# JzHuai0108/sim3opt

Hardware: AMD Instinct MI355X
Metric: LM iterations/s (higher is better)
Workload: dtype f64

## Files before the change

sim3opt_amd/csrc/amg_kernels.hpp:

```cpp
#pragma once

__global__ __launch_bounds__(WG) void k_amg_adjoint(int nb, const int32_t* __restrict__ row2v,
                                                    const Sim3* __restrict__ states,
                                                    double* __restrict__ P) {
  for (int i = blockIdx.x * WG + threadIdx.x; i < nb; i += gridDim.x * WG) {
  const Sim3 S = load_sim3(states + row2v[i]);
  double R[9];
  sim3::R_from_quat(S.q, R);
  double A[49];
#pragma unroll
  for (int k = 0; k < 49; ++k) A[k] = 0.0;
  const double t0 = S.t[0], t1 = S.t[1], t2 = S.t[2];
#pragma unroll
  for (int c = 0; c < 3; ++c) {
    const double v0 = R[c], v1 = R[3 + c], v2 = R[6 + c];
    A[0 + 7 * c] = v0;
    A[1 + 7 * c] = v1;
    A[2 + 7 * c] = v2;
    A[3 + 7 * c] = t1 * v2 - t2 * v1;
    A[4 + 7 * c] = t2 * v0 - t0 * v2;
    A[5 + 7 * c] = t0 * v1 - t1 * v0;
    A[3 + 7 * (3 + c)] = S.s * v0;
    A[4 + 7 * (3 + c)] = S.s * v1;
    A[5 + 7 * (3 + c)] = S.s * v2;
  }
  A[3 + 42] = -t0;
  A[4 + 42] = -t1;
  A[5 + 42] = -t2;
  A[6 + 42] = 1.0;
  double* dst = P + (size_t)49 * i;
#pragma unroll
  for (int k = 0; k < 49; ++k) dst[k] = A[k];
  }
}

template <bool HASP>
__global__ __launch_bounds__(WG) void k_amg_galerkin(int cb0, int cb1, const int32_t* __restrict__ gptr,
                                                     const int32_t* __restrict__ gblk,
                                                     const int32_t* __restrict__ grow,
                                                     const int32_t* __restrict__ colidx_f,
                                                     const double* __restrict__ vals_f,
                                                     const double* __restrict__ P,
                                                     double* __restrict__ vals_c,
                                                     float* __restrict__ vals32_f) {
  const int lane = threadIdx.x & 63;
  const int cb = cb0 + __builtin_amdgcn_readfirstlane((int)(blockIdx.x * 4 + (threadIdx.x >> 6)));
  if (cb >= cb1) return;
  const int l49 = lane < 49 ? lane : lane - 49;
  const int r = l49 % 7, c = l49 / 7;
  double acc = 0.0;
  const int e0 = gptr[cb], e1 = gptr[cb + 1];
  for (int eb = e0; eb < e1; eb += 64) {
    const int n = e1 - eb < 64 ? e1 - eb : 64;
    const int le = lane < n ? lane : n - 1;
    const int kkv = gblk[eb + le];
    if (HASP) {
      const int giv = grow[eb + le];
      const int cjv = colidx_f[kkv];
      double av[2], pj[2][7], pi[2][7];
      int kk[2];
      auto load = [&](int u, int b) {
        kk[b] = __builtin_amdgcn_readlane(kkv, u);
        av[b] = vals_f[(size_t)49 * kk[b] + l49];
        const double* pjp = P + (size_t)49 * __builtin_amdgcn_readlane(cjv, u) + 7 * c;
        const double* pip = P + (size_t)49 * __builtin_amdgcn_readlane(giv, u) + 7 * r;
#pragma unroll
        for (int q = 0; q < 7; ++q) {
          pj[b][q] = pjp[q];
          pi[b][q] = pip[q];
        }
      };
      auto consume = [&](int b) {
        if (vals32_f && lane < 49) vals32_f[f32_pair_index(kk[b], lane)] = (float)av[b];
        double t = 0.0;
#pragma unroll
        for (int q = 0; q < 7; ++q) t += __shfl(av[b], r + 7 * q) * pj[b][q];
        double o = 0.0;
#pragma unroll
        for (int q = 0; q < 7; ++q) o += pi[b][q] * __shfl(t, q + 7 * c);
        acc += o;
      };
      for (int u = 0; u < n; ++u) {
        load(u, 0);
        consume(0);
      }
    } else {
      for (int u0 = 0; u0 < n; u0 += 4) {
        const int m = n - u0 < 4 ? n - u0 : 4;
        int kk[4];
        double av[4];
#pragma unroll
        for (int u = 0; u < 4; ++u)
          if (u < m) {
            kk[u] = __builtin_amdgcn_readlane(kkv, u0 + u);
            av[u] = vals_f[(size_t)49 * kk[u] + l49];
          }
#pragma unroll
        for (int u = 0; u < 4; ++u)
          if (u < m) {
            if (vals32_f && lane < 49) vals32_f[f32_pair_index(kk[u], lane)] = (float)av[u];
            acc += av[u];
          }
      }
    }
  }
  if (lane < 49) vals_c[(size_t)49 * cb + lane] = acc;
}

__global__ __launch_bounds__(WG) void k_amg_copydiag(int lo, int hi, const int32_t* __restrict__ rowptr,
                                                     const double* __restrict__ vals,
                                                     double* __restrict__ diagH) {
  for (int idx = 49 * lo + blockIdx.x * WG + threadIdx.x; idx < 49 * hi; idx += gridDim.x * WG)
    diagH[idx] = vals[(size_t)49 * rowptr[idx / 49] + idx % 49];
}

// ... 19 lines not shown
      acc += v;
    }
  }
  if (lane < 49) Wc[(size_t)49 * a + lane] = acc;
}


template <int K>
__global__ __launch_bounds__(WG) void k_amg_restrict(int a_lo, int nc, const int32_t* __restrict__ mptr,
                                                     const int32_t* __restrict__ mem,
                                                     const double* __restrict__ t_f,
                                                     double* __restrict__ r_c,
                                                     const double* __restrict__ Minv_c,
                                                     double* __restrict__ x_c, int64_t vs_f, int64_t vs_c,
                                                     int64_t ms_c) {
  const int lane = threadIdx.x & 63;
  const int wave = threadIdx.x >> 6;
  const int sub = lane / 7, rr = lane % 7, base = lane - rr;
  if (gridDim.y > 1) {
    const size_t s0 = (size_t)blockIdx.y * K;
    t_f += s0 * vs_f;
    r_c += s0 * vs_c;
    x_c += s0 * vs_c;
    if (Minv_c) Minv_c += s0 * ms_c;
  }
  for (int a0 = a_lo + (blockIdx.x * 4 + wave) * 9; a0 < nc; a0 += gridDim.x * 36) {
    const int a = a0 + sub;
    const bool act = lane < 63 && a < nc;
    const int e0 = act ? mptr[a] : 0, e1 = act ? mptr[a + 1] : 0;
#pragma unroll
    for (int s = 0; s < K; ++s) {
      const double* tf = t_f + (size_t)s * vs_f;
      double acc = 0.0;
      int e = e0;
      for (; e + 3 < e1; e += 4) {
        const int i0 = mem[e], i1 = mem[e + 1], i2 = mem[e + 2], i3 = mem[e + 3];
        const double v0 = tf[(size_t)7 * i0 + rr], v1 = tf[(size_t)7 * i1 + rr];
        const double v2 = tf[(size_t)7 * i2 + rr], v3 = tf[(size_t)7 * i3 + rr];
        acc += (v0 + v1) + (v2 + v3);
      }
      for (; e < e1; ++e) acc += tf[(size_t)7 * mem[e] + rr];
      if (act) r_c[(size_t)s * vs_c + (size_t)7 * a + rr] = acc;
      if (Minv_c) {
        double xv = 0.0;
#pragma unroll
        for (int cc = 0; cc < 7; ++cc) {
          const double rc = __shfl(acc, base + cc);
          if (act) xv += Minv_c[(size_t)s * ms_c + (size_t)49 * a + 7 * rr + cc] * rc;
        }
        if (act) x_c[(size_t)s * vs_c + (size_t)7 * a + rr] = xv;
      }
    }
  }
}

template <int K>
__device__ inline bool all_done(const DevScalars* __restrict__ sc) {
  bool done = sc != nullptr;
#pragma unroll
  for (int s = 0; s < K; ++s) done = done && sc[s].done;
  return done;
}

template <int K>
__global__ __launch_bounds__(WG) void k_amg_restrict0(int a_lo, int nc, const int32_t* __restrict__ mptr,
                                                      const int32_t* __restrict__ mem,
                                                      const double* __restrict__ P,
                                                      const double* __restrict__ t_f,
                                                      double* __restrict__ r_c,
                                                      const double* __restrict__ Minv_c,
                                                      double* __restrict__ x_c,
                                                      const DevScalars* __restrict__ sc, int64_t vs_f, int64_t vs_c,
                                                      int64_t ms_c) {
  if (all_done<K>(sc)) return;
  const int lane = threadIdx.x & 63;
  const int a = a_lo + __builtin_amdgcn_readfirstlane((int)(blockIdx.x * 4 + (threadIdx.x >> 6)));
  if (a >= nc) return;
  const int l49 = lane < 49 ? lane : lane - 49;
  const int m = l49 % 7, c = l49 / 7;
  double acc[K];
#pragma unroll
  for (int s = 0; s < K; ++s) acc[s] = 0.0;
  const int e0 = mptr[a], e1 = mptr[a + 1];
  for (int e = e0; e < e1; ++e) {
    const int i = mem[e];
    const double pv = P[(size_t)49 * i + l49];
#pragma unroll
    for (int s = 0; s < K; ++s) acc[s] += pv * t_f[(size_t)s * vs_f + (size_t)7 * i + m];
  }
#pragma unroll
  for (int s = 0; s < K; ++s) {
    double rc = 0.0;
#pragma unroll
    for (int q = 0; q < 7; ++q) rc += __shfl(acc[s], 7 * c + q);
    if (lane < 49 && m == 0) r_c[(size_t)s * vs_c + (size_t)7 * a + c] = rc;
    if (Minv_c) {
      const double pr = Minv_c[(size_t)s * ms_c + (size_t)49 * a + l49] * rc;
      double xv = pr;
#pragma unroll
      for (int q = 1; q < 7; ++q) xv += __shfl(pr, m + 7 * ((c + q) % 7));
      if (lane < 7) x_c[(size_t)s * vs_c + (size_t)7 * a + lane] = xv;
    }
  }
}

__global__ __launch_bounds__(WG) void k_amg_bjapply(int nb, const double* __restrict__ Minv,
                                                    const double* __restrict__ r,
                                                    double* __restrict__ x) {
  const int lane = threadIdx.x & 63;
  const int wave = threadIdx.x >> 6;
  const int sub = lane / 7, rr = lane % 7, base = lane - rr;
  for (int row0 = (blockIdx.x * 4 + wave) * 9; row0 < nb; row0 += gridDim.x * 36) {
    const int row = row0 + sub;
    const bool act = lane < 63 && row < nb;
    const double rv = act ? r[(size_t)7 * row + rr] : 0.0;
    double xv = 0.0;
#pragma unroll
    for (int cc = 0; cc < 7; ++cc) {
      const double rc = __shfl(rv, base + cc);
      if (act) xv += Minv[(size_t)49 * row + 7 * rr + cc] * rc;
    }
    if (act) x[(size_t)7 * row + rr] = xv;
  }
}

template <bool HASP, int K>
__global__ __launch_bounds__(WG) void k_amg_prolong(int row_lo, int row_hi, const int32_t* __restrict__ list,
                                                    const int32_t* __restrict__ agg,
                                                    const double* __restrict__ P,
                                                    const double* __restrict__ x_c,
                                                    const double* x_in, double* x_out,
                                                    const DevScalars* __restrict__ sc, double scale, int64_t vs_f,
                                                    int64_t vs_c) {
  if (all_done<K>(sc)) return;
  const int lane = threadIdx.x & 63;
  const int wave = threadIdx.x >> 6;
  const int sub = lane / 7, rr = lane % 7, base = lane - rr;
  for (int row0 = row_lo + (blockIdx.x * 4 + wave) * 9; row0 < row_hi; row0 += gridDim.x * 36) {
    const bool act = lane < 63 && row0 + sub < row_hi;
    const int row = act ? (list ? list[row0 + sub] : row0 + sub) : 0;
    const int ag = act ? agg[row] : 0;
    constexpr bool HOIST = HASP && K > 1;
    double pm[HOIST ? 7 : 1];
    if constexpr (HOIST) {
#pragma unroll
      for (int m = 0; m < 7; ++m) pm[m] = act ? P[(size_t)49 * row + rr + 7 * m] : 0.0;
    }
#pragma unroll
    for (int s = 0; s < K; ++s) {
      const double xc = act ? x_c[(size_t)s * vs_c + (size_t)7 * ag + rr] : 0.0;
      double add = xc;
      if constexpr (HASP) {
        add = 0.0;
#pragma unroll
        for (int m = 0; m < 7; ++m) {
          const double xm = __shfl(xc, base + m);
          if constexpr (HOIST) {
            if (act) add += pm[m] * xm;
          } else {
            if (act) add += P[(size_t)49 * row + rr + 7 * m] * xm;
          }
        }
      }
      const size_t j = (size_t)s * vs_f + (size_t)7 * row + rr;
      if (act) x_out[j] = x_in[j] + scale * add;
    }
  }
}

constexpr int AMG_DENSE_MAX_N = 7 * AMG_MAX_COARSEST;
__global__ __launch_bounds__(WG) void k_amg_dense_fill(int nb, const int32_t* __restrict__ rowptr,
                                                       const int32_t* __restrict__ colidx,
                                                       const double* __restrict__ vals,
                                                       double* __restrict__ A,
                                                       const double* __restrict__ diag64 = nullptr) {
  const int n = 7 * nb;
  const int nnz = 49 * rowptr[nb];
  for (int t = blockIdx.x * WG + threadIdx.x; t < nnz; t += gridDim.x * WG) {
    const int k = t / 49, e = t % 49;
    int lo = 0, hi = nb;
    while (hi - lo > 1) {
      const int mid = (lo + hi) >> 1;
      if (rowptr[mid] <= k) lo = mid; else hi = mid;
    }
    const double v = diag64 && k == rowptr[lo] ? diag64[(size_t)49 * lo + e] : vals[(size_t)49 * k + e];
    A[(size_t)(7 * lo + e % 7) * n + 7 * colidx[k] + e / 7] = v;
  }
}


template <int NP>
__device__ inline bool gj_invert_rows(double (&prow)[NP], int lane) {
  bool spd = true;
#pragma unroll
  for (int k = 0; k < NP; ++k) {
    double pk[NP];
#pragma unroll
    for (int c = 0; c < NP; ++c) pk[c] = __shfl(prow[c], k);
    if (!(pk[k] > 0.0)) spd = false;
    const double d = 1.0 / pk[k];
    const double f = prow[k];
#pragma unroll
    for (int j = 0; j < NP; ++j) {
      const double rk = pk[j] * d;
      if (lane == k) prow[j] = j == k ? d : rk;
      else prow[j] = j == k ? -f * d : prow[j] - f * rk;
    }
  }
  return spd;
}

template <int NP>
__device__ inline bool gj_invert_halfrows(double (&prow)[NP / 2], int lane) {
  constexpr int H = NP / 2;
  const int r = lane & 31, h = lane >> 5;
  bool spd = true;
#pragma unroll
  for (int k = 0; k < NP; ++k) {
    const int hk = k / H, kk = k % H;
    double pk[H];
#pragma unroll
    for (int c = 0; c < H; ++c) pk[c] = __shfl(prow[c], k + 32 * h);
    const double pkk = __shfl(prow[kk], k + 32 * hk);
    if (!(pkk > 0.0)) spd = false;
    const double d = 1.0 / pkk;
    const double f = __shfl(prow[kk], r + 32 * hk);
#pragma unroll
    for (int j = 0; j < H; ++j) {
      const double rk = pk[j] * d;
      const bool pivcol = j == kk && h == hk;
      if (r == k) prow[j] = pivcol ? d : rk;
      else prow[j] = pivcol ? -f * d : prow[j] - f * rk;
    }
  }
  return spd;
}

template <int NP>
__device__ inline void gj_invert_block(const double* src, int ld, double* __restrict__ Pout, int lane,
                                       DevScalars* sc) {
  bool spd;
  if constexpr (NP % 2 == 0) {
    constexpr int H = NP / 2;
    double prow[H];
// ... 166 lines not shown
```

sim3opt_amd/csrc/engine_amg.hip:

```cpp
#include "engine_impl.hpp"

#include <cassert>

namespace sim3opt {

#include "spmv_kernel.hpp"
#include "amg_kernels.hpp"

int Engine::amg_init(const Structure& s, bool automatic, std::string& err) {
  (void)err;
  amg_omega = std::max(0.1, std::min(0.95, opt.amg_omega));
  amg_additive = opt.amg_additive != 0;
  {
    const bool partitioned = part_world() >= 2;
    int last = 0;
    for (int l = 1; l <= AMG_MAX_LEVELS; ++l) {
      const int o = l <= 4 ? opt.amg_cycle[l - 1] : 0;
      if (o >= 1 && o <= 3) last = o;
      amg_visits[l] = last > 0 ? last : (partitioned ? (l <= 1 ? 1 : 2) : (l <= 1 ? 2 : 3));
    }
    amg_visits[0] = 1;
  }
  amg_fp32 = opt.amg_fp32 != 0;
  adaptive_prec = opt.adaptive_prec != 0 && automatic;
  amg_pivot = opt.amg_pivot >= 28 ? 28 : 14;
  for (int l = 0; l <= AMG_MAX_LEVELS; ++l)
    amg_over_l[l] = std::max(0.5, std::min(3.0, l == 0 ? opt.amg_over[0] : opt.amg_over[1]));
  std::string why;
  AmgBuildOptions bo;
  bo.max_coarsest = opt.amg_coarsest;
  for (int k = 0; k < 3; ++k) bo.passes[k] = opt.amg_passes[k];
  std::vector<int32_t> vbegin;
  bo.world = part_world();
  bo.shard_rows = std::max(1, opt.amg_shard_rows);
  if (comm.world > 1) {
    bo.row_begin = row_begin.data();
  } else if (bo.world > 1) {
    vbegin.resize(bo.world + 1);
    partition_rows_equal(nb, bo.world, vbegin.data());
    bo.row_begin = vbegin.data();
  }
  if (!build_amg_hierarchy(nb, s.rowptr.data(), s.colidx.data(), amg_host, why, bo)) {
    if (opt.verbose) std::fprintf(stderr, "sim3opt: no multigrid hierarchy (%s)\n", why.c_str());
    amg_host.clear();
    return SIM3OPT_OK;
  }
  if (automatic && (double)amg_host[1].nnzb > 0.3 * (double)amg_host[0].nnzb) {
    if (opt.verbose)
      std::fprintf(stderr, "sim3opt: the graph coarsens like an expander (level-1 blocks %.2f of level 0): block-Jacobi\n",
                   (double)amg_host[1].nnzb / (double)amg_host[0].nnzb);
    amg_host.clear();
    return SIM3OPT_OK;
  }
  use_amg = true;
  return SIM3OPT_OK;
}

int Engine::amg_bind(const Structure& s, std::string& err) {
  std::vector<AmgLevelHost>& H = amg_host;
  const int nl = (int)H.size();
  amg.assign(nl, AmgLevel());
  int rc = SIM3OPT_OK;
#define AMGCHK(call) do { rc = (call); if (rc) return rc; } while (0)
  AmgLevel& L0 = amg[0];
  L0.nb = nb; L0.nnzb = nnzb;
  L0.rowptr = d_rowptr; L0.colidx = d_colidx; L0.wrow = d_wrow; L0.span_grid = span_grid;
  L0.vals = d_vals; L0.Minv = d_Minv; L0.r = d_r; L0.x = d_z;
  int64_t padded = 0;
  (void)allgather_equal_plan(offs.data(), comm.world, nullptr, &padded);
  HIPCHK(mem.alloc(d_az, std::max<size_t>((size_t)n, (size_t)padded), nullptr));
  HIPCHK(mem.alloc(d_P, (size_t)49 * nb, nullptr));
  HIPCHK(upload(d_row2v, s.row2vertex));
  L0.t = d_az;
  L0.lo = r0; L0.hi = r1;
  const int64_t shard_rows = std::max(1, opt.amg_shard_rows);
  rep_level = 1;
  while (rep_level < nl - 1 && H[rep_level].nb > shard_rows && !H[rep_level].row_begin.empty() &&
         H[rep_level].respects_owner)
    ++rep_level;
  if (comm.active()) {
    parts.resize(rep_level);
    n_sharded = rep_level;
  }
  for (int l = 0; l < nl; ++l) {
    AmgLevel& L = amg[l];
    const AmgLevelHost& h = H[l];
    if (l > 0) {
      L.nb = h.nb; L.nnzb = h.nnzb;
      L.lo = 0; L.hi = L.nb;
      HIPCHK(upload(L.rowptr, h.rowptr));
      HIPCHK(upload(L.colidx, h.colidx));
      if (sharded(l)) {
        AMGCHK(level_part_init(l, L.nb, h.rowptr.data(), h.colidx.data(), h.row_begin, err));
        L.lo = parts[l].lo; L.hi = parts[l].hi;
      }
      const int nloc = L.hi - L.lo;
      L.span_grid = std::max(1, (nloc + 3) / 4);
      std::vector<int32_t> wrow(L.span_grid * 4 + 1);
      partition_rows(nloc, h.rowptr.data() + L.lo, L.span_grid * 4, wrow.data());
      for (int32_t& w : wrow) w += L.lo;
      HIPCHK(upload(L.wrow, wrow));
      AMGCHK(alloc_ranged(L.vals, 49 * (int64_t)h.rowptr[L.lo], 49 * (int64_t)h.rowptr[L.hi], 49 * (int64_t)L.nnzb, err));
      HIPCHK(mem.alloc(L.diagH, (size_t)49 * L.nb, nullptr));
      HIPCHK(mem.alloc(L.W, (size_t)49 * L.nb, nullptr));
      HIPCHK(mem.alloc(L.Minv, (size_t)49 * L.nb, nullptr));
      HIPCHK(mem.alloc(L.r, (size_t)7 * L.nb, nullptr));
      HIPCHK(mem.alloc(L.x, (size_t)7 * L.nb, nullptr));
      HIPCHK(mem.alloc(L.t, (size_t)7 * L.nb, nullptr));
    }
    if (amg_fp32) {
      const int64_t b0 = l == 0 ? s.rowptr[L.lo] : h.rowptr[L.lo], b1 = l == 0 ? s.rowptr[L.hi] : h.rowptr[L.hi];
      const int64_t n32 = 98 * ((std::max<int64_t>(L.nnzb, 1) + 1) / 2);
      AMGCHK(alloc_ranged(L.vals32, 98 * (b0 / 2), 98 * ((b1 + 1) / 2), n32, err));
    }
    if (l + 1 < nl) {
      HIPCHK(upload(L.agg, h.agg));
      HIPCHK(upload(L.mptr, h.mptr));
      HIPCHK(upload(L.mem, h.mem));
      HIPCHK(upload(L.gptr, h.gptr));
      HIPCHK(upload(L.gblk, h.gblk));
      HIPCHK(upload(L.grow, h.grow));
    }
  }
  const size_t nc = (size_t)7 * amg[nl - 1].nb;
  HIPCHK(mem.alloc(d_Ainv, nc * nc, nullptr));
  HIPCHK(mem.alloc(d_Ainv2, nc * nc, nullptr));
  HIPCHK(mem.alloc(d_piv, 2 * 28 * 28, nullptr));
#undef AMGCHK
  lvl_offs.assign(nl, std::vector<int64_t>());
  lvl_blk_offs.assign(nl, std::vector<int64_t>());
  for (int l = 1; l < nl; ++l) {
    amg[l].own_lo = 0; amg[l].own_hi = amg[l].nb;
    if (sharded(l - 1)) {
      const std::vector<int32_t> rb = H[l].row_begin.empty() ? std::vector<int32_t>{0, H[l].nb} : H[l].row_begin;
      amg[l].own_lo = rb[comm.rank];
      amg[l].own_hi = rb[comm.rank + 1];
      lvl_offs[l].resize(comm.world + 1);
      lvl_blk_offs[l].resize(comm.world + 1);
      for (int r = 0; r <= comm.world; ++r) {
        lvl_offs[l][r] = 7 * (int64_t)rb[r];
        lvl_blk_offs[l][r] = 49 * (int64_t)H[l].rowptr[rb[r]];
      }
    }
    amg[l].own_b0 = H[l].rowptr[amg[l].own_lo];
    amg[l].own_b1 = H[l].rowptr[amg[l].own_hi];
  }
  if (opt.verbose) {
    std::fprintf(stderr, "sim3opt: multigrid levels (rows/blocks):");
    for (const AmgLevel& L : amg) std::fprintf(stderr, " %d/%lld", L.nb, (long long)L.nnzb);
    if (comm.active()) std::fprintf(stderr, "; levels 0..%d partitioned over the ranks, the rest replicated", n_sharded - 1);
    std::fprintf(stderr, "; visits of levels 1, 2, 3: %d %d %d\n", amg_visits[1], amg_visits[2], amg_visits[3]);
  }
  cv_one = CycleView();
  cv_one.lv.resize(nl);
  for (int l = 0; l < nl; ++l) {
    cv_one.lv[l].Minv = amg[l].Minv;
    cv_one.lv[l].r = amg[l].r;
    cv_one.lv[l].x = amg[l].x;
    cv_one.lv[l].t = amg[l].t;
  }
  cv_one.sc = d_sc;
  cv_one.Ainv = d_Ainv;
  cv_one.rz_part = d_part_b;
  amg_host.clear();
  amg_host.shrink_to_fit();
  amg_stale = true;
  return SIM3OPT_OK;
}

int Engine::amg_setup(std::string& err) {
  const int nl = (int)amg.size();
  hipLaunchKernelGGL(k_amg_adjoint, dim3(grid_for(nb, WG)), dim3(WG), 0, stream, nb, d_row2v,
                     d_states, d_P);
  for (int l = 0; l + 1 < nl; ++l) {
    const AmgLevel& F = amg[l];
    AmgLevel& Cc = amg[l + 1];
    const int cb0 = (int)Cc.own_b0, cb1 = (int)Cc.own_b1;
    const int gg = std::max(1, (cb1 - cb0 + 3) / 4), gw = (Cc.nb + 3) / 4;
    if (l == 0)
      hipLaunchKernelGGL((k_amg_galerkin<true>), dim3(gg), dim3(WG), 0, stream, cb0, cb1, F.gptr,
                         F.gblk, F.grow, F.colidx, F.vals, d_P, Cc.vals, amg_fp32 ? F.vals32 : (float*)nullptr);
    else
      hipLaunchKernelGGL((k_amg_galerkin<false>), dim3(gg), dim3(WG), 0, stream, cb0, cb1, F.gptr,
                         F.gblk, F.grow, F.colidx, F.vals, (const double*)nullptr, Cc.vals,
                         amg_fp32 ? F.vals32 : (float*)nullptr);
    if (comm.active() && sharded(l) && !sharded(l + 1)) {
      int rc = comm.allgatherv(Cc.vals, lvl_blk_offs[l + 1], stream, err);
      if (rc) return rc;
    }
    if (l == 0)
      hipLaunchKernelGGL((k_amg_wsum<true>), dim3(gw), dim3(WG), 0, stream, Cc.nb, F.mptr, F.mem, d_P, Cc.W);
    else
      hipLaunchKernelGGL((k_amg_wsum<false>), dim3(gw), dim3(WG), 0, stream, Cc.nb, F.mptr, F.mem, F.W, Cc.W);
    hipLaunchKernelGGL(k_amg_copydiag, dim3(grid_for(49 * (int64_t)std::max(1, Cc.hi - Cc.lo), WG)), dim3(WG), 0, stream,
                       Cc.lo, Cc.hi, Cc.rowptr, Cc.vals, Cc.diagH);
  }
  if (amg_fp32)
    for (int l = nl - 1; l < nl; ++l) {
      const size_t cnt = (size_t)49 * (size_t)amg[l].nnzb;
      hipLaunchKernelGGL(k_to_f32, dim3(grid_for((int64_t)(cnt / 4), WG)), dim3(WG), 0, stream, cnt,
                         (const double*)amg[l].vals, amg[l].vals32);
    }
  HIPCHK(hipGetLastError());
  amg_stale = false;
  return SIM3OPT_OK;
}

void Engine::amg_prepare(double lambda) {
  const int nl = (int)amg.size();
  for (int l = 0; l < nl; ++l) {
    const AmgLevel& L = amg[l];
    const int lo = L.lo, hi = L.hi;
    jacobi(lo, hi, L.rowptr, L.vals, lambda, L.Minv, l == 0 && amg_additive ? 1.0 : amg_omega, L.diagH, L.W,
           l > 0 ? L.vals32 : (float*)nullptr);
  }
  dense_inverse(nullptr, d_Ainv, d_sc);
}

void Engine::dense_inverse(const double* diag64, double* Aout, DevScalars* sc) {
  const int nl = (int)amg.size();
  const AmgLevel& Lc = amg[nl - 1];
  const int nd = 7 * Lc.nb;
  auto pivot_rows = [&](int k0) { return nd - k0 >= amg_pivot ? amg_pivot : (nd - k0 >= 14 ? 14 : 7); };
  int nsteps = 0;
  for (int k0 = 0; k0 < nd; k0 += pivot_rows(k0)) ++nsteps;
  double *src = nsteps % 2 ? d_Ainv2 : Aout, *dst = nsteps % 2 ? Aout : d_Ainv2;
  (void)hipMemsetAsync(src, 0, sizeof(double) * (size_t)nd * nd, stream);
  hipLaunchKernelGGL(k_amg_dense_fill, dim3(grid_for(49 * Lc.nnzb, WG)), dim3(WG), 0, stream, Lc.nb,
                     Lc.rowptr, Lc.colidx, Lc.vals, src, diag64);
  double *pin = d_piv, *pout = d_piv + 28 * 28;
  switch (pivot_rows(0)) {
    case 28: hipLaunchKernelGGL((k_amg_dense_gj_first<28>), dim3(1), dim3(64), 0, stream, nd, (const double*)src, pin, sc); break;
    case 14: hipLaunchKernelGGL((k_amg_dense_gj_first<14>), dim3(1), dim3(64), 0, stream, nd, (const double*)src, pin, sc); break;
    default: hipLaunchKernelGGL((k_amg_dense_gj_first<7>), dim3(1), dim3(64), 0, stream, nd, (const double*)src, pin, sc);
  }
  const dim3 gt((nd + 63) / 64, (nd + 63) / 64 + 1);
  for (int k0 = 0; k0 < nd;) {
    const int pb = pivot_rows(k0), pbn = k0 + pb < nd ? pivot_rows(k0 + pb) : 0;
    if (pb == 28)
      hipLaunchKernelGGL((k_amg_dense_gj_step<28>), gt, dim3(WG), 0, stream, nd, k0, (const double*)src,
                         dst, (const double*)pin, pout, pbn, sc);
    else if (pb == 14)
      hipLaunchKernelGGL((k_amg_dense_gj_step<14>), gt, dim3(WG), 0, stream, nd, k0, (const double*)src,
                         dst, (const double*)pin, pout, pbn, sc);
    else
      hipLaunchKernelGGL((k_amg_dense_gj_step<7>), gt, dim3(WG), 0, stream, nd, k0, (const double*)src,
                         dst, (const double*)pin, pout, pbn, sc);
    k0 += pb;
    std::swap(src, dst);
    std::swap(pin, pout);
  }
}

void Engine::spmv_mode(const CycleView& V, int level, int mode, const double* v, double* out, const double* xc) {
  const AmgLevel& L = amg[level];
  const CycleLevel& B = V.lv[level];
  DevScalars* const sc = level == 0 ? V.sc : nullptr;
  double* const rz_part = level == 0 && mode == 2 && !amg_additive ? V.rz_part : nullptr;
  const BatchStrides bs{B.vs, B.ms, level + 1 < (int)amg.size() ? V.lv[level + 1].vs : 0, B.ms, V.part};
#define PASS(CHV, NTV, MODEV, VT, KV, DIAGV, SLICES, VALS)                                                           \
  hipLaunchKernelGGL((k_spmv_span<CHV, NTV, MODEV, VT, KV, DIAGV>), dim3(L.span_grid, SLICES), dim3(WG), 0, stream, \
                     L.nb, L.wrow, L.rowptr, L.colidx, (const VT*)(VALS), v, out, 0.0, rz_part, B.r,                 \
                     const_cast<double*>(xc), sc, (const double*)B.Minv, 1, (const int32_t*)L.agg, amg_over, bs,     \
                     (const float*)B.diag32)
#define PASS_FINE(CHV, VT, KV, VALS) \
  do { if (mode == 1) PASS(CHV, true, 1, VT, KV, false, 1, VALS); else PASS(CHV, true, 2, VT, KV, false, 1, VALS); } while (0)
#define PASS_COARSE(CHV, VT, KV, DIAGV, SLICES, VALS)                 \
  do {                                                                \
    if (mode == 1) PASS(CHV, false, 1, VT, KV, DIAGV, SLICES, VALS);  \
    else if (mode == 3) PASS(CHV, false, 3, VT, KV, DIAGV, SLICES, VALS); \
    else PASS(CHV, false, 2, VT, KV, DIAGV, SLICES, VALS);            \
  } while (0)
  if (!V.batch) {
    if (amg_fp32) {
      if (level == 0) PASS_FINE(F32_CH, float, 1, L.vals32); else PASS_COARSE(COARSE_CH, float, 1, false, 1, L.vals32);
    } else {
      if (level == 0) PASS_FINE(8, double, 1, L.vals); else PASS_COARSE(8, double, 1, false, 1, L.vals);
    }
  } else if (level == 0) {
    BATCH_DISPATCH(V.nsys, PASS_FINE(F32_CH, float, KS, L.vals32));
  } else if (L.nnzb <= b_slice_blocks) {
    PASS_COARSE(8, float, 1, true, V.nsys, L.vals32);
  } else {
    BATCH_DISPATCH(V.nsys, PASS_COARSE(8, float, KS, true, 1, L.vals32));
  }
#undef PASS_COARSE
#undef PASS_FINE
#undef PASS
}

void Engine::amg_restrict(const CycleView& V, int l, const double* t) {
  const AmgLevel& F = amg[l];
  const AmgLevel& Cc = amg[l + 1];
  const CycleLevel &BF = V.lv[l], &BC = V.lv[l + 1];
  const int a0 = Cc.own_lo, a1 = Cc.own_hi;
  const bool gather = comm.active() && sharded(l) && !sharded(l + 1);
  const double* Minv_c = l + 2 < (int)amg.size() ? BC.Minv : nullptr;
  const double* Minv_k = gather ? nullptr : Minv_c;
  if (l == 0)
    BATCH_DISPATCH(V.nsys, hipLaunchKernelGGL((k_amg_restrict0<KS>), dim3(std::max(1, (a1 - a0 + 3) / 4)), dim3(WG), 0,
                       stream, a0, a1, F.mptr, F.mem, d_P, t, BC.r, Minv_k, BC.x, (const DevScalars*)V.sc, BF.vs,
                       BC.vs, BC.ms));
  else
    hipLaunchKernelGGL((k_amg_restrict<1>), dim3(grid_for((a1 - a0 + 8) / 9, 4), V.nsys), dim3(WG), 0, stream, a0, a1,
                       F.mptr, F.mem, t, BC.r, Minv_k, BC.x, BF.vs, BC.vs, BC.ms);
  if (gather) {
    if (amg_status == SIM3OPT_OK) amg_status = comm.allgatherv(BC.r, lvl_offs[l + 1], stream, amg_err);
    if (Minv_c)
      hipLaunchKernelGGL(k_amg_bjapply, dim3(grid_for((Cc.nb + 8) / 9, 4)), dim3(WG), 0, stream, Cc.nb, Minv_c,
                         (const double*)BC.r, BC.x);
  }
}

void Engine::amg_prolong(const CycleView& V, int l, const double* xc, const double* xin, double* xout) {
  const AmgLevel& F = amg[l];
  const DevScalars* scp = l == 0 ? V.sc : nullptr;
  const int64_t vs_f = V.lv[l].vs, vs_c = V.lv[l + 1].vs;
  auto rows = [&](int lo, int hi, const int32_t* list) {
    const int g = grid_for((hi - lo + 8) / 9, 4);
    if (l == 0)
      BATCH_DISPATCH(V.nsys, hipLaunchKernelGGL((k_amg_prolong<true, KS>), dim3(g), dim3(WG), 0, stream, lo, hi, list,
                         F.agg, d_P, xc, xin, xout, scp, amg_over, vs_f, vs_c));
    else
      BATCH_DISPATCH(V.nsys, hipLaunchKernelGGL((k_amg_prolong<false, KS>), dim3(g), dim3(WG), 0, stream, lo, hi, list,
                         F.agg, (const double*)nullptr, xc, xin, xout, scp, amg_over, vs_f, vs_c));
  };
  rows(F.lo, F.hi, nullptr);
  if (comm.active() && sharded(l) && !parts[l].neighbour)
    amg_exchange(l, xout);
  else if (comm.active() && sharded(l) && parts[l].n_recv > 0 && !parts[l].self_test)
    rows(0, parts[l].n_recv, parts[l].d_recv);
}

void Engine::amg_exchange(int l, double* vec) {
  if (!comm.active() || !sharded(l)) return;
  if (amg_status == SIM3OPT_OK) amg_status = exchange_level(l, vec, amg_err);
}

double* Engine::amg_coarse(const CycleView& V, int l) {
  if (opt.time_kernels && l + 1 == rep_level && part_world() > 1 && !V.batch) {
    if (rep_used + 2 > rep_pool.size()) {
      hipEvent_t e0 = nullptr, e1 = nullptr;
      if (event_acquire(&e0) == hipSuccess && event_acquire(&e1) == hipSuccess) {
        rep_pool.push_back(e0);
        rep_pool.push_back(e1);
      }
    }
    if (rep_used + 2 <= rep_pool.size()) {
      (void)hipEventRecord(rep_pool[rep_used], stream);
      double* res = amg_coarse_body(V, l);
      (void)hipEventRecord(rep_pool[rep_used + 1], stream);
      rep_used += 2;
      return res;
    }
  }
  return amg_coarse_body(V, l);
}

double* Engine::amg_coarse_body(const CycleView& V, int l) {
  const int nl = (int)amg.size();
  const AmgLevel& Cc = amg[l + 1];
  const CycleLevel& BC = V.lv[l + 1];
  if (l + 2 == nl) {
    hipLaunchKernelGGL((k_amg_dense_apply<1>), dim3(std::max(1, std::min(256, (7 * Cc.nb + 3) / 4)), V.nsys), dim3(WG),
                       0, stream, 7 * Cc.nb, (const double*)V.Ainv, (const double*)BC.r, BC.x, V.as, BC.vs);
    return BC.x;
  }
  amg_exchange(l + 1, BC.x);
  double* res = amg_cycle(V, l + 1, BC.x, BC.t);
  for (int g = 1; g < amg_visits[l + 1]; ++g) {
    double* oth = res == BC.x ? BC.t : BC.x;
    amg_exchange(l + 1, res);
    spmv_mode(V, l + 1, 2, res, oth);
    amg_exchange(l + 1, oth);
    res = amg_cycle(V, l + 1, oth, res);
  }
  return res;
}

double* Engine::amg_cycle(const CycleView& V, int l, double* cur, double* other) {
  assert(!V.batch || (amg_fp32 && !amg_additive && !comm.active()));
  spmv_mode(V, l, 1, cur, other);
  amg_restrict(V, l, other);
  double* xc = amg_coarse(V, l);
  amg_exchange(l + 1, xc);
  amg_over = amg_over_on ? amg_over_l[l] : 1.0;
  if (l == 0) {
    amg_prolong(V, l, xc, cur, cur);
    spmv_mode(V, l, 2, cur, other);
  } else {
    spmv_mode(V, l, 3, cur, other, xc);
  }
  return other;
}

int Engine::amg_apply(std::string& err) {
  amg_status = SIM3OPT_OK;
  if (amg_additive) {
    amg_restrict(cv_one, 0, d_r);
    double* xc0 = amg_coarse(cv_one, 0);
    amg_exchange(1, xc0);
    amg_over = amg_over_on ? amg_over_l[0] : 1.0;
    amg_prolong(cv_one, 0, xc0, d_z, d_az);
  } else {
    amg_exchange(0, d_z);
// ... 93 lines not shown
```

sim3opt_amd/csrc/engine_impl.hpp:

```cpp
#pragma once
#include <hip/hip_runtime.h>
#include <hip/hip_ext.h>

#include <algorithm>
#include <cfloat>
#include <chrono>
#include <cmath>
#include <cstdio>
#include <cstddef>
#include <cstdlib>
#include <cstring>

#include "amg.hpp"
#include "comm.hpp"
#include "devmem.hpp"
#include "direct_factor.hpp"
#include "engine.hpp"

namespace sim3opt {

using sim3::Sim3;

constexpr int COARSE_CH = 8;
constexpr int F32_CH = 8;
// ... 61 lines not shown
    const double ga = g[a];
    if (!(ga > 0.0) || !(gb > 0.0) || !(gb < ga) || !(target > 0.0)) return -1.0;
    if (gb <= target) return 0.0;
    const double x = (double)(k[n - 1] - k[a]) * std::log(target / gb) / std::log(gb / ga);
    return std::isfinite(x) ? std::max(x, 0.0) : -1.0;
  }
};

#include "dev_common.hpp"
struct EdgeArgs;

static inline int64_t pad64(int64_t n) { return (n + 63) / 64 * 64; }
static inline int grid_for(int64_t items, int per_block) {
  const int64_t g = (items + per_block - 1) / per_block;
  return (int)std::max<int64_t>(1, std::min<int64_t>(g, MAX_GRID));
}

class Engine {
 public:
  sim3opt_options opt;
  Structure st;
  int32_t nv = 0, ne = 0, nb = 0, n = 0, n_active = 0;
  int64_t nnzb = 0;
  bool has_info = false, has_kernel = false;
  hipStream_t stream = nullptr;
  DevArena mem;
  template <typename T>
  hipError_t upload(T*& dptr, const std::vector<T>& h) { return mem.upload(dptr, h, stream, &staged); }
  Sim3 *d_states = nullptr, *d_backup = nullptr, *d_meas = nullptr;
  int32_t *d_ev0 = nullptr, *d_ev1 = nullptr, *d_hidx = nullptr, *d_active = nullptr;
  double *d_info = nullptr, *d_kdelta = nullptr;
  uint8_t* d_kkind = nullptr;
  int32_t *d_rowptr = nullptr, *d_colidx = nullptr, *d_incptr = nullptr, *d_wrow = nullptr;
  int span_grid = 0;
  int32_t *d_slot01 = nullptr, *d_slot10 = nullptr, *d_inc0 = nullptr, *d_inc1 = nullptr;
  double *d_vals = nullptr, *d_scratch = nullptr, *d_b = nullptr, *d_Minv = nullptr;
  struct RangedArray { void* alloc; size_t elem; int64_t total, lo, hi; };
  std::vector<RangedArray> ranged;
  template <typename T>
  int alloc_ranged(T*& virt, int64_t lo, int64_t hi, int64_t total, std::string& err) {
    total = std::max<int64_t>(total, 1);
    lo = std::max<int64_t>(0, std::min(lo, total));
    hi = std::max(lo, std::min(hi, total));
    T* p = nullptr;
    if (opt.debug_full_arrays) {
      HIPCHK(mem.raw(p, (size_t)total));
      HIPCHK(hipMemset(p, 0xFF, sizeof(T) * (size_t)total));
      if (hi > lo) HIPCHK(hipMemset(p + lo, 0, sizeof(T) * (size_t)(hi - lo)));
      virt = p;
    } else {
      HIPCHK(mem.alloc(p, (size_t)(hi - lo), nullptr));
      virt = reinterpret_cast<T*>(reinterpret_cast<uintptr_t>(p) - sizeof(T) * (size_t)lo);
    }
    ranged.push_back({p, sizeof(T), total, lo, hi});
    return SIM3OPT_OK;
  }
  int check_foreign_ranges(std::string& err);
  int64_t ranged_bytes() const {
    int64_t b = 0;
    for (const RangedArray& a : ranged) b += (int64_t)a.elem * (opt.debug_full_arrays ? a.total : std::max<int64_t>(a.hi - a.lo, 1));
    return b;
  }
  double *d_x = nullptr, *d_r = nullptr, *d_z = nullptr, *d_p = nullptr, *d_q = nullptr, *d_s = nullptr;
  double *d_part_a = nullptr, *d_part_b = nullptr;
  int32_t *d_sub_first = nullptr, *d_sub_cnt = nullptr;
  double* d_Gm = nullptr;
  bool use_chain = false;
  int chain_seg = 256;
  struct AmgLevel {
    int32_t nb = 0;
    int64_t nnzb = 0;
    int32_t *rowptr = nullptr, *colidx = nullptr, *wrow = nullptr;
    int span_grid = 0;
    double *vals = nullptr, *diagH = nullptr, *W = nullptr, *Minv = nullptr;
    float* vals32 = nullptr;
    int32_t *agg = nullptr, *mptr = nullptr, *mem = nullptr, *gptr = nullptr, *gblk = nullptr, *grow = nullptr;
    double *r = nullptr, *x = nullptr, *t = nullptr;
    int32_t lo = 0, hi = 0;
    int32_t own_lo = 0, own_hi = 0;
    int64_t own_b0 = 0, own_b1 = 0;
  };
  std::vector<std::vector<int64_t>> lvl_offs, lvl_blk_offs;
  std::vector<AmgLevel> amg;
  double *d_P = nullptr, *d_Ainv = nullptr, *d_Ainv2 = nullptr, *d_piv = nullptr, *d_az = nullptr;
  int32_t* d_row2v = nullptr;
  bool use_amg = false, amg_stale = true;
  double amg_omega = 0.9;
  int amg_visits[AMG_MAX_LEVELS + 1];
  bool amg_additive = false;
  bool amg_fp32 = true;
  double amg_over_l[AMG_MAX_LEVELS + 1];
  double amg_over = 1.0;
  bool amg_over_on = true;
  int amg_pivot = 14;
  bool adaptive_prec = true;
  double bj_gate = -1.0;
  int bj_budget = 48;
  int n_bj_solves = 0, n_bj_abandoned = 0;
  bool trace_stale = true;
  double mean_diag = 0.0;
  int amg_status = 0;
  std::string amg_err;
  struct CycleLevel {
    double *Minv = nullptr, *r = nullptr, *x = nullptr, *t = nullptr;
    float* diag32 = nullptr;
    int64_t vs = 0, ms = 0;
  };
  struct CycleView {
    int nsys = 1;
    bool batch = false;
    std::vector<CycleLevel> lv;
    DevScalars* sc = nullptr;
    double* Ainv = nullptr;
    int64_t as = 0;
    double* rz_part = nullptr;
    int part = 0;
  };
  CycleView cv_one;
  CycleView cv_batch;
  struct PcgView {
    int nsys = 1;
    int nsc = 1;
    bool batch = false;
    double *x = nullptr, *r = nullptr, *z = nullptr, *p = nullptr, *q = nullptr, *s = nullptr, *az = nullptr;
    int64_t vs = 0;
    double* Minv = nullptr;
    int64_t ms = 0;
    const double* b = nullptr;
    int64_t bstride = 0;
    double tol[KB] = {0, 0, 0, 0}, lam[KB] = {0, 0, 0, 0};
    DevScalars *sc = nullptr, *h_sc = nullptr;
    double *part_a = nullptr, *part_b = nullptr;
    int pstride = 0;
    CycleView* cv = nullptr;
  };
  PcgView pv_one;
  PcgView pv_batch;
  DevArena batch_mem;
  double *b_x = nullptr, *b_r = nullptr, *b_z = nullptr, *b_p = nullptr, *b_q = nullptr, *b_s = nullptr, *b_az = nullptr;
  double *b_Ainv = nullptr, *b_diag64 = nullptr, *b_part_a = nullptr, *b_part_b = nullptr;
  int64_t b_vs = 0, b_as = 0;
  DevScalars *d_bsc = nullptr, *h_bsc = nullptr;
  bool batch_ready = false;
  int64_t b_slice_blocks = 100000;
  int batch_alloc(std::string& err);
  void batch_release();
  void batch_prepare(int nsetup);
  struct BatchRhs { const double* g; int64_t stride; const double* tol; bool setup; };
  int pcg_batch(const double* lams, int nsys, int32_t* iters, double* rel_res, bool* capped, bool* usable,
                std::string& err, const BatchRhs* cols = nullptr);
  int lm_trial_solve(int q, double lambda, double ni, const double** x, int32_t* iters, double* rel_res, bool* ok,
                     std::string& err);
  struct TrialBatch {
    int n = 0, next = 0;
    double lam[KB], rel[KB];
    int32_t iters[KB], prev_pit = 0;
    bool capped[KB], prev_ok = false, prev_capped = false;
  } trial_batch;
  int batch_capacity() const {
    if (!use_amg || use_direct || comm.active() || !amg_fp32 || amg_additive || opt.pcg_batch == 1) return 0;
    return opt.pcg_batch > 1 ? std::min(opt.pcg_batch, KB) : KB;
  }
  BlockLdl lm_factor;
  bool use_direct = false;
  int fail_token = 1;
  bool chi_known = false;
  double chi_cache = 0.0;
// ... 229 lines not shown
```

Before: 50.80.

## Store compact 16-double pose records and rebuild prolongator entries on the fly

Setup now writes a 16-double pose record (rotation, translation, scale) per block alongside the full 49-double prolongator. The level-0 restriction and prolongation kernels read the compact record and recompute P entries in registers, using lane shuffles in restrict and per-row selection in prolong. This cuts the bytes read per block in the hot cycle kernels, at the cost of extra arithmetic and shuffles. The restrict loop is also unrolled over 2 or 4 aggregate members to expose more loads at once.

Result: no change. 50.72 (median of 2 runs) (-0.2%).

```diff
diff --git a/sim3opt_amd/csrc/amg_kernels.hpp b/sim3opt_amd/csrc/amg_kernels.hpp
--- a/sim3opt_amd/csrc/amg_kernels.hpp
+++ b/sim3opt_amd/csrc/amg_kernels.hpp
@@ -1,36 +1,96 @@
 #pragma once
 
-__global__ __launch_bounds__(WG) void k_amg_adjoint(int nb, const int32_t* __restrict__ row2v,
-                                                    const Sim3* __restrict__ states,
-                                                    double* __restrict__ P) {
+constexpr int AMG_REC = 16;
+constexpr int AMG_REC_USED = 13;
+
+template <class Rec>
+__device__ __forceinline__ double amg_p_entry(Rec rec, int r, int c) {
+  S3_STRICT_FP
+  const int k = r - 3, a = k == 2 ? 0 : k + 1, b = k == 0 ? 2 : k - 1;
+  const bool mid = r >= 3 && r < 6;
+  const bool rot = r < 3 && c < 3, cross = mid && c < 3, scaled = mid && c >= 3 && c < 6, negt = mid && c == 6;
+  const int s1 = cross ? 9 + a : scaled ? 12 : rot ? 3 * r + c : negt ? 9 + k : 0;
+  const int s2 = cross ? 3 * b + c : scaled ? 3 * k + c - 3 : 0;
+  const int s3 = cross ? 9 + b : 0, s4 = cross ? 3 * a + c : 0;
+  const double x1 = rec(s1), y1 = rec(s2), x2 = rec(s3), y2 = rec(s4);
+  const double sub = x2 * y2;
+  const double cr = __builtin_fma(x1, y1, -sub);
+  const double sc = x1 * y1;
+  return cross ? cr : scaled ? sc : rot ? x1 : negt ? -x1 : (r == 6 && c == 6 ? 1.0 : 0.0);
+}
+
+__device__ __forceinline__ int amg_rec_lane(int lane) {
+  const int s = lane & (AMG_REC - 1);
+  return s < AMG_REC_USED ? s : AMG_REC_USED - 1;
+}
+
+__device__ __forceinline__ double amg_p_entry_lanes(double slotv, int r, int c) {
+  return amg_p_entry([&](int s) { return __shfl(slotv, s); }, r, c);
+}
+
+struct AmgPose {
+  double r0, r1, r2, r3, r4, r5, r6, r7, r8, t0, t1, t2, s;
+  __device__ __forceinline__ double operator()(int slot) const {
+    switch (slot) {
+      case 0: return r0;
+      case 1: return r1;
+      case 2: return r2;
+      case 3: return r3;
+      case 4: return r4;
+      case 5: return r5;
+      case 6: return r6;
+      case 7: return r7;
+      case 8: return r8;
+      case 9: return t0;
+      case 10: return t1;
+      case 11: return t2;
+      default: return s;
+    }
+  }
+};
+__device__ __forceinline__ AmgPose amg_pose_load(const double* __restrict__ p) {
+  return AmgPose{p[0], p[1], p[2], p[3], p[4], p[5], p[6], p[7], p[8], p[9], p[10], p[11], p[12]};
+}
+__device__ __forceinline__ double amg_sel3(int k, double x, double y, double z) {
+  return k == 0 ? x : k == 1 ? y : z;
+}
+
+__device__ __forceinline__ void amg_p_row(const AmgPose& u, int r, double (&row)[7]) {
+  const int k = r < 3 ? r : r < 6 ? r - 3 : 0;
+  const AmgPose p{amg_sel3(k, u.r0, u.r3, u.r6), amg_sel3(k, u.r1, u.r4, u.r7), amg_sel3(k, u.r2, u.r5, u.r8),
+                  amg_sel3(k, u.r3, u.r6, u.r0), amg_sel3(k, u.r4, u.r7, u.r1), amg_sel3(k, u.r5, u.r8, u.r2),
+                  amg_sel3(k, u.r6, u.r0, u.r3), amg_sel3(k, u.r7, u.r1, u.r4), amg_sel3(k, u.r8, u.r2, u.r5),
+                  amg_sel3(k, u.t0, u.t1, u.t2), amg_sel3(k, u.t1, u.t2, u.t0), amg_sel3(k, u.t2, u.t0, u.t1),
+                  u.s};
+#pragma unroll
+  for (int m = 0; m < 7; ++m) {
+    const double e0 = amg_p_entry(p, 0, m), e3 = amg_p_entry(p, 3, m), e6 = amg_p_entry(p, 6, m);
+    row[m] = r < 3 ? e0 : r < 6 ? e3 : e6;
+  }
+}
+
+template <int... E>
+__device__ __forceinline__ void amg_p_expand(const AmgPose& u, double* __restrict__ blk, std::integer_sequence<int, E...>) {
+  ((blk[E] = amg_p_entry(u, E % 7, E / 7)), ...);
+}
+
+__global__ __launch_bounds__(WG) void k_amg_pose_record(int nb, const int32_t* __restrict__ row2v,
+                                                        const Sim3* __restrict__ states,
+                                                        double* __restrict__ rec, double* __restrict__ P) {
   for (int i = blockIdx.x * WG + threadIdx.x; i < nb; i += gridDim.x * WG) {
-  const Sim3 S = load_sim3(states + row2v[i]);
-  double R[9];
-  sim3::R_from_quat(S.q, R);
-  double A[49];
-#pragma unroll
-  for (int k = 0; k < 49; ++k) A[k] = 0.0;
-  const double t0 = S.t[0], t1 = S.t[1], t2 = S.t[2];
-#pragma unroll
-  for (int c = 0; c < 3; ++c) {
-    const double v0 = R[c], v1 = R[3 + c], v2 = R[6 + c];
-    A[0 + 7 * c] = v0;
-    A[1 + 7 * c] = v1;
-    A[2 + 7 * c] = v2;
-    A[3 + 7 * c] = t1 * v2 - t2 * v1;
-    A[4 + 7 * c] = t2 * v0 - t0 * v2;
-    A[5 + 7 * c] = t0 * v1 - t1 * v0;
-    A[3 + 7 * (3 + c)] = S.s * v0;
-    A[4 + 7 * (3 + c)] = S.s * v1;
-    A[5 + 7 * (3 + c)] = S.s * v2;
-  }
-  A[3 + 42] = -t0;
-  A[4 + 42] = -t1;
-  A[5 + 42] = -t2;
-  A[6 + 42] = 1.0;
-  double* dst = P + (size_t)49 * i;
-#pragma unroll
-  for (int k = 0; k < 49; ++k) dst[k] = A[k];
+    const Sim3 S = load_sim3(states + row2v[i]);
+    double R[9];
+    sim3::R_from_quat(S.q, R);
+    const AmgPose u{R[0], R[1], R[2], R[3], R[4], R[5], R[6], R[7], R[8], S.t[0], S.t[1], S.t[2], S.s};
+    double* dst = rec + (size_t)AMG_REC * i;
+#pragma unroll
+    for (int k = 0; k < 9; ++k) dst[k] = R[k];
+    dst[9] = u.t0;
+    dst[10] = u.t1;
+    dst[11] = u.t2;
+    dst[12] = u.s;
+    dst[13] = dst[14] = dst[15] = 0.0;
+    amg_p_expand(u, P + (size_t)49 * i, std::make_integer_sequence<int, 49>());
   }
 }
 
@@ -216,11 +276,26 @@
 #pragma unroll
   for (int s = 0; s < K; ++s) acc[s] = 0.0;
   const int e0 = mptr[a], e1 = mptr[a + 1];
-  for (int e = e0; e < e1; ++e) {
-    const int i = mem[e];
-    const double pv = P[(size_t)49 * i + l49];
-#pragma unroll
-    for (int s = 0; s < K; ++s) acc[s] += pv * t_f[(size_t)s * vs_f + (size_t)7 * i + m];
+  const int ls = amg_rec_lane(lane);
+  constexpr int U = K == 1 ? 4 : 2;
+  for (int e = e0; e < e1; e += U) {
+    const int n = e1 - e < U ? e1 - e : U;
+    double rv[U], tv[U][K];
+#pragma unroll
+    for (int u = 0; u < U; ++u) {
+      const int i = mem[e + (u < n ? u : n - 1)];
+      rv[u] = P[(size_t)AMG_REC * i + ls];
+#pragma unroll
+      for (int s = 0; s < K; ++s) tv[u][s] = t_f[(size_t)s * vs_f + (size_t)7 * i + m];
+    }
+#pragma unroll
+    for (int u = 0; u < U; ++u) {
+      const double pv = amg_p_entry_lanes(rv[u], m, c);
+      if (u < n) {
+#pragma unroll
+        for (int s = 0; s < K; ++s) acc[s] += pv * tv[u][s];
+      }
+    }
   }
 #pragma unroll
   for (int s = 0; s < K; ++s) {
@@ -274,11 +349,9 @@
     const bool act = lane < 63 && row0 + sub < row_hi;
     const int row = act ? (list ? list[row0 + sub] : row0 + sub) : 0;
     const int ag = act ? agg[row] : 0;
-    constexpr bool HOIST = HASP && K > 1;
-    double pm[HOIST ? 7 : 1];
-    if constexpr (HOIST) {
-#pragma unroll
-      for (int m = 0; m < 7; ++m) pm[m] = act ? P[(size_t)49 * row + rr + 7 * m] : 0.0;
+    double pm[HASP ? 7 : 1];
+    if constexpr (HASP) {
+      amg_p_row(amg_pose_load(P + (size_t)AMG_REC * row), rr, pm);
     }
 #pragma unroll
     for (int s = 0; s < K; ++s) {
@@ -289,11 +362,7 @@
 #pragma unroll
         for (int m = 0; m < 7; ++m) {
           const double xm = __shfl(xc, base + m);
-          if constexpr (HOIST) {
-            if (act) add += pm[m] * xm;
-          } else {
-            if (act) add += P[(size_t)49 * row + rr + 7 * m] * xm;
-          }
+          if (act) add += pm[m] * xm;
         }
       }
       const size_t j = (size_t)s * vs_f + (size_t)7 * row + rr;
diff --git a/sim3opt_amd/csrc/engine_amg.hip b/sim3opt_amd/csrc/engine_amg.hip
--- a/sim3opt_amd/csrc/engine_amg.hip
+++ b/sim3opt_amd/csrc/engine_amg.hip
@@ -69,6 +69,7 @@
   int64_t padded = 0;
   (void)allgather_equal_plan(offs.data(), comm.world, nullptr, &padded);
   HIPCHK(mem.alloc(d_az, std::max<size_t>((size_t)n, (size_t)padded), nullptr));
+  HIPCHK(mem.alloc(d_prec, (size_t)AMG_REC * nb, nullptr));
   HIPCHK(mem.alloc(d_P, (size_t)49 * nb, nullptr));
   HIPCHK(upload(d_row2v, s.row2vertex));
   L0.t = d_az;
@@ -170,8 +171,8 @@
 
 int Engine::amg_setup(std::string& err) {
   const int nl = (int)amg.size();
-  hipLaunchKernelGGL(k_amg_adjoint, dim3(grid_for(nb, WG)), dim3(WG), 0, stream, nb, d_row2v,
-                     d_states, d_P);
+  hipLaunchKernelGGL(k_amg_pose_record, dim3(grid_for(nb, WG)), dim3(WG), 0, stream, nb, d_row2v,
+                     d_states, d_prec, d_P);
   for (int l = 0; l + 1 < nl; ++l) {
     const AmgLevel& F = amg[l];
     AmgLevel& Cc = amg[l + 1];
@@ -299,7 +300,7 @@
   const double* Minv_k = gather ? nullptr : Minv_c;
   if (l == 0)
     BATCH_DISPATCH(V.nsys, hipLaunchKernelGGL((k_amg_restrict0<KS>), dim3(std::max(1, (a1 - a0 + 3) / 4)), dim3(WG), 0,
-                       stream, a0, a1, F.mptr, F.mem, d_P, t, BC.r, Minv_k, BC.x, (const DevScalars*)V.sc, BF.vs,
+                       stream, a0, a1, F.mptr, F.mem, d_prec, t, BC.r, Minv_k, BC.x, (const DevScalars*)V.sc, BF.vs,
                        BC.vs, BC.ms));
   else
     hipLaunchKernelGGL((k_amg_restrict<1>), dim3(grid_for((a1 - a0 + 8) / 9, 4), V.nsys), dim3(WG), 0, stream, a0, a1,
@@ -320,7 +321,7 @@
     const int g = grid_for((hi - lo + 8) / 9, 4);
     if (l == 0)
       BATCH_DISPATCH(V.nsys, hipLaunchKernelGGL((k_amg_prolong<true, KS>), dim3(g), dim3(WG), 0, stream, lo, hi, list,
-                         F.agg, d_P, xc, xin, xout, scp, amg_over, vs_f, vs_c));
+                         F.agg, d_prec, xc, xin, xout, scp, amg_over, vs_f, vs_c));
     else
       BATCH_DISPATCH(V.nsys, hipLaunchKernelGGL((k_amg_prolong<false, KS>), dim3(g), dim3(WG), 0, stream, lo, hi, list,
                          F.agg, (const double*)nullptr, xc, xin, xout, scp, amg_over, vs_f, vs_c));
diff --git a/sim3opt_amd/csrc/engine_impl.hpp b/sim3opt_amd/csrc/engine_impl.hpp
--- a/sim3opt_amd/csrc/engine_impl.hpp
+++ b/sim3opt_amd/csrc/engine_impl.hpp
@@ -167,7 +167,7 @@
   };
   std::vector<std::vector<int64_t>> lvl_offs, lvl_blk_offs;
   std::vector<AmgLevel> amg;
-  double *d_P = nullptr, *d_Ainv = nullptr, *d_Ainv2 = nullptr, *d_piv = nullptr, *d_az = nullptr;
+  double *d_prec = nullptr, *d_P = nullptr, *d_Ainv = nullptr, *d_Ainv2 = nullptr, *d_piv = nullptr, *d_az = nullptr;
   int32_t* d_row2v = nullptr;
   bool use_amg = false, amg_stale = true;
   double amg_omega = 0.9;
```
